# sandialabs/calibr8

Hardware: AMD Instinct MI355X
Metric: element Jacobian assemblies/sec, 1M hex8 J2-plasticity fp64 (higher is better)
Workload: dtype f64

## Files before the change

### calibr8_amd/csrc/c8_assemble_node.hpp

```cpp
#pragma once

#include "c8_assemble_wave.hpp"

#ifdef C8_STAMPS
#define C8_NSTAMP(i) ex.stamp_node(ga.stamps, node, i)
#else
#define C8_NSTAMP(i)
#endif

namespace c8 {

template <class M, class = void> struct has_closed_form_rows : std::false_type {};
template <class M> struct has_closed_form_rows<M, std::enable_if_t<M::HAS_CLOSED_FORM_ROWS>> : std::true_type {};

template <class E, class ModelD, int MAXDEG, bool MANY> struct NodeShared {
  static constexpr int NR = ModelD::NROW;
  static constexpr int LDR = NR + 4;
  static_assert(LDR % 2 == 0 && (E::NP0 * LDR * 8) % 256 == 128, "record stride: 16-byte aligned, element groups 32 banks apart");
  static constexpr int NREC = 8 * E::NP0 * LDR, NACC = MAXDEG * 16;
  alignas(16) double buf[MANY ? NREC + NACC : (NREC > NACC ? NREC : NACC)];
  alignas(16) double nodal[8][E::NN][4];
  double nshape[8];
  double el[8][2];
  double bsum[4];
  C8_HD double* rec(int s, int pt) { return buf + (s * E::NP0 + pt) * LDR; }
  C8_HD double* img() { return buf + (MANY ? NREC : 0); }
  C8_HD static int img01(int deg) { return 9 * deg; }
  C8_HD static int img10(int deg) { return 12 * deg; }
  C8_HD static int img11(int deg) { return 15 * deg; }
};

C8_HD double const* at_byte(double const* p, int off) { return reinterpret_cast<double const*>(reinterpret_cast<char const*>(p) + off); }

constexpr int NODE_NXI = 7;
template <int MAXDEG> struct NodeLane {
  static constexpr int N00 = (9 * MAXDEG + 63) / 64, N01 = (3 * MAXDEG + 63) / 64;
  double J[16];
  double a00[N00], a01[N01], a10[N01], a11;
  double bold;
  double rs;
  double G[9], xo[NODE_NXI], w, h;
  int e, a, pos;
  bool valid;
};

template <class EX, class = void> struct has_xor8 : std::false_type {};
template <class EX> struct has_xor8<EX, std::void_t<typename EX::has_xor8>> : std::true_type {};
template <class EX, class = void> struct has_lane_marker : std::false_type {};
template <class EX> struct has_lane_marker<EX, std::void_t<decltype(std::declval<EX&>().cur)>> : std::true_type {};
template <int C, class EX, class F> C8_HD double lane_xor8(EX& ex, int lane, F get) {
  static_assert(C >= 0 && C < 8, "partner inside the group of eight lanes");
  if constexpr (C == 0) return get(lane);
  else if constexpr (has_xor8<EX>::value) return ex.template xor8<C>(lane, get);
  else if constexpr (has_lane_marker<EX>::value) {
    int const saved = ex.cur;
    ex.cur = lane ^ C;
    double const v = get(lane ^ C);
    ex.cur = saved;
    return v;
  } else return get(lane ^ C);
}

C8_HD constexpr int hex_code(int n) { return n ^ ((n >> 1) & 1); }
template <class E> C8_HD void hex_pattern(int j, double* v) {
  double c[3], w;
  E::point(0, 7, c, w);
  double const a = 1. + ((j & 1) ? c[0] : -c[0]), b = 1. + ((j & 2) ? c[1] : -c[1]), d = 1. + ((j & 4) ? c[2] : -c[2]);
  v[0] = 0.125 * a * b * d;
  v[1] = 0.125 * b * d;
  v[2] = 0.125 * a * d;
  v[3] = 0.125 * a * b;
}

template <class E> struct HexShape {
  double c[3];
  C8_HD static HexShape of_point(int pt) {
    double w;
    HexShape h;
    E::point(0, pt, h.c, w);
    return h;
  }
  C8_HD double at_node(int n) const {
    double const sx = ((n ^ (n >> 1)) & 1) ? 1. : -1., sy = ((n >> 1) & 1) ? 1. : -1., sz = ((n >> 2) & 1) ? 1. : -1.;
    return 0.125 * (1. + sx * c[0]) * (1. + sy * c[1]) * (1. + sz * c[2]);
  }
};

template <class E, template <class> class ModelT, int MAXDEG, bool MANY, bool ADJ = false, class EX>
C8_HD void node_rows_closed(EX& ex, NodeShared<E, ModelT<Dual>, MAXDEG, MANY>& sh, MeshTables const& mt, ModelSettings const& ms,
                            FieldArgs const& fa, GatherArgs const& ga, int node, AdjointArgs const& aa = AdjointArgs{}) {
  using Model = ModelT<Dual>;
  using SH = NodeShared<E, Model, MAXDEG, MANY>;
  using NL_ = NodeLane<MAXDEG>;
  constexpr int NL = Model::NLOC, NR = SH::NR;
  static_assert(NL <= NODE_NXI, "NodeLane::xo holds a point's local state");
  static_assert(E::NN == 8 && E::NP0 == 8 && E::SAME_POINTS, "row-per-node kernel: hex8-like element");
  static_assert(!Mechanics::USES_U && !Model::FINITE_DEF, "row-per-node kernel: small-strain weak form without u terms");
  C8_NSTAMP(6);
  int const nptr = ga.nodeptr[node], deg = ga.nodeptr[node + 1] - nptr;
  int const e0 = ga.nodeelem_ptr[node], e1 = ga.nodeelem_ptr[node + 1];
  size_t const np = (size_t)nptr;
  int const n3 = 3 * deg;
  if (e0 == e1) return;
  C8_NSTAMP(0);
  auto zero_acc = [&](int lane) {
    C8_UNROLL
    for (int it = 0; it < (SH::NACC + 63) / 64; ++it) {
      int const q = lane + 64 * it;
      if (q < 16 * deg) sh.img()[q] = 0.;
    }
    if (lane < 4) sh.bsum[lane] = 0.;
  };
  if (!ADJ || MANY) {
    ex.each([&](int lane) {
      if (!ADJ && lane < 8) {
        double v[4];
        hex_pattern<E>(lane, v);
        sh.nshape[lane] = v[0];
      }
      if (MANY) zero_acc(lane);
    });
    ex.sync();
  }
  for (int c0 = e0; c0 < e1; c0 += 8) {
    int const ne = (e1 - c0 < 8) ? e1 - c0 : 8;
    ex.each([&](int lane) {
      auto& r = ex.lane(lane);
      int const s = lane >> 3, m = lane & 7, mp = hex_code(m);
      r.valid = s < ne;
      r.rs = 0.;
      if (!r.valid) return;
      int const packed = ga.nodeelem[c0 + s];
      int const e = packed >> 3, a = packed & 7;
      r.e = e;
      r.a = a;
      int const nd = mt.conn[(size_t)e * E::NN + m];
      r.pos = ga.pos[((size_t)e * E::NN + m) * E::NN + a];
      {
        double const* const t = mt.shape + (size_t)e * SHAPE_STRIDE;
        C8_UNROLL
        for (int c = 0; c < 9; ++c) r.G[c] = t[SHAPE_JINV + 8 * c + mp];
        if constexpr (!ADJ) {
          size_t const q0 = ((size_t)e * E::NP0 + mp) * NL;
          C8_UNROLL
          for (int j = 0; j < NL; ++j) r.xo[j] = fa.xi_prev[q0 + j];
        }
        r.w = t[SHAPE_WDV + mp];
        r.h = t[SHAPE_H];
      }
      double* const nv = sh.nodal[s][m];
      nv[0] = fa.u[(size_t)nd * 3 + 0]; nv[1] = fa.u[(size_t)nd * 3 + 1]; nv[2] = fa.u[(size_t)nd * 3 + 2];
      nv[3] = fa.p[nd];
    });
    ex.sync();
    ex.each([&](int lane_) {
      auto& r = ex.lane(lane_);
      int lane = lane_;
      C8_PIN(lane);
      int const s = lane >> 3, pt = hex_code(lane & 7);
      if (!r.valid) return;
      int const e = r.e, a = r.a;
      size_t const q0 = ((size_t)e * E::NP0 + pt) * NL;
      double G[9], xi_old[NL];
      C8_UNROLL
      for (int c = 0; c < 9; ++c) G[c] = r.G[c];
      if constexpr (!ADJ) {
        C8_UNROLL
        for (int j = 0; j < NL; ++j) xi_old[j] = r.xo[j];
      }
      double fh4[4] = {0., 0., 0., 0.}, gx[NL];
      C8_UNROLL
      for (int j = 0; j < NL; ++j) gx[j] = 0.;
      if constexpr (ADJ) {
        double const* const fh = aa.f + ((size_t)e * E::NP0 + pt) * E::NDOF;
        fh4[0] = fh[3 * a + 0]; fh4[1] = fh[3 * a + 1]; fh4[2] = fh[3 * a + 2]; fh4[3] = fh[3 * E::NN + a];
        C8_UNROLL
        for (int j = 0; j < NL; ++j) gx[j] = aa.g[((size_t)e * E::NP0 + pt) * NL + j];
      }
      double q[WQ];
      C8_UNROLL
      for (int c = 0; c < WQ; ++c) q[c] = 0.;
      double g[3];
      {
        double R[12], pN = 0.;
        C8_UNROLL
        for (int c = 0; c < 12; ++c) R[c] = 0.;
        int const mo = hex_code(pt ^ 7) * 32;
        C8_UNROLL
        for (int i = 0; i < E::NN; ++i) {
          double v[4];
          hex_pattern<E>(i, v);
          double const t0 = (i & 1) ? v[1] : -v[1], t1 = (i & 2) ? v[2] : -v[2], t2 = (i & 4) ? v[3] : -v[3];
          double const* const nv = at_byte(sh.nodal[s][0], mo ^ (hex_code(i) * 32));
          double const u0 = nv[0], u1 = nv[1], u2 = nv[2], pm = nv[3];
          R[0] += u0 * t0; R[1] += u0 * t1; R[2] += u0 * t2;
          R[3] += u1 * t0; R[4] += u1 * t1; R[5] += u1 * t2;
          R[6] += u2 * t0; R[7] += u2 * t1; R[8] += u2 * t2;
          pN += pm * v[0];
          R[9] += pm * t0; R[10] += pm * t1; R[11] += pm * t2;
        }
        double const s0 = (pt & 1) ? 1. : -1., s1 = (pt & 2) ? 1. : -1., s2 = (pt & 4) ? 1. : -1.;
        C8_UNROLL
        for (int f = 0; f < 4; ++f) {
          double const r0 = s0 * R[3 * f], r1 = s1 * R[3 * f + 1], r2 = s2 * R[3 * f + 2];
          C8_UNROLL
          for (int d = 0; d < 3; ++d) q[(f < 3 ? 3 * f : 10) + d] = r0 * G[d] + r1 * G[3 + d] + r2 * G[6 + d];
        }
        q[9] = pN;
        double xa[3], wa, da[3];
        E::point(0, pt, xa, wa);
        E::dNdxi(a, xa, da);
        C8_UNROLL
        for (int d = 0; d < 3; ++d) g[d] = da[0] * G[d] + da[1] * G[3 + d] + da[2] * G[6 + d];
      }
      C8_NSTAMP(7);
      if constexpr (ADJ) {
        C8_UNROLL
        for (int j = 0; j < NL; ++j) xi_old[j] = fa.xi_prev[q0 + j];
      }
      int const es = mt.elem_set ? mt.elem_set[e] : 0;
      C8_UNROLL
      for (int c = 0; c < 9; ++c) r.G[c] = ((pt >> (c / 3)) & 1) ? G[c] : -G[c];
      typename Model::ClosedForm cf;
      Model::closed_form(mt.params + (size_t)es * Model::NPARAMS, q, xi_old, ms.abs_tol, r.h, ms.stab_mult, cf, true);
      if (!ADJ && a == 0) {
        C8_UNROLL
        for (int j = 0; j < NL; ++j) fa.xi[q0 + j] = cf.xi[j];
      }
      C8_NSTAMP(8);
      double const w = r.w;
      double Na;
      if constexpr (ADJ) Na = HexShape<E>::of_point(pt).at_node(a);
      else Na = sh.nshape[hex_code(a) ^ pt ^ 7];
      double* const rc = sh.rec(s, pt);
      double el[2];
      Model::template closed_form_row<ADJ>(cf.t, w, g, Na, rc, el);
      if (pt == 0) { sh.el[s][0] = el[0]; sh.el[s][1] = el[1]; }
      if constexpr (!ADJ) {
        C8_UNROLL
        for (int i = 0; i < 3; ++i) rc[NR + i] = w * (cf.F[3 * i] * g[0] + cf.F[3 * i + 1] * g[1] + cf.F[3 * i + 2] * g[2]);
        rc[NR + 3] = w * (cf.F[9] * Na + cf.F[10] * g[0] + cf.F[11] * g[1] + cf.F[12] * g[2]);
      } else {
        double Re[6];
        double dq[10];
        C8_UNROLL
        for (int k = 0; k < 10; ++k) dq[k] = 0.;
        if (aa.qoi.c_load != 0.) {
          double dxi[NL];
          Model::closed_form_load_term(mt.params + (size_t)es * Model::NPARAMS, aa.qoi.c_load * w, aa.qoi.comp,
                                       aa.qoi.S + ((size_t)e * E::NP0 + pt) * 3, dxi, dq);
          C8_UNROLL
          for (int j = 0; j < NL; ++j) gx[j] -= dxi[j];
        }
        Model::closed_form_adjoint(mt.params + (size_t)es * Model::NPARAMS, cf.t, gx, Re);
        double const dJ = aa.qoi.c_avg * w / aa.qoi.ndims * Na;
        rc[NR + 0] = (Re[0] - dq[0]) * g[0] + (Re[1] - dq[1]) * g[1] + (Re[2] - dq[2]) * g[2] - dJ + fh4[0];
        rc[NR + 1] = (Re[1] - dq[3]) * g[0] + (Re[3] - dq[4]) * g[1] + (Re[4] - dq[5]) * g[2] - dJ + fh4[1];
        rc[NR + 2] = (Re[2] - dq[6]) * g[0] + (Re[4] - dq[7]) * g[1] + (Re[5] - dq[8]) * g[2] - dJ + fh4[2];
        rc[NR + 3] = -dq[9] * Na + fh4[3];
      }
    });
    ex.sync();
    C8_NSTAMP(1);
    ex.each([&](int lane_) {
      auto& r = ex.lane(lane_);
      int lane = lane_;
      C8_PIN(lane);
      C8_UNROLL
      for (int j = 0; j < 16; ++j) r.J[j] = 0.;
      if (!r.valid) return;
      int const s = lane >> 3, m = lane & 7;
      double const el[2] = {sh.el[s][0], sh.el[s][1]};
      auto step = [&](auto cc) {
        constexpr int c = decltype(cc)::value, hc = hex_code(c);
        double v[4];
        hex_pattern<E>(hc ^ 7, v);
        double const k0 = (hc & 1) ? -v[1] : v[1], k1 = (hc & 2) ? -v[2] : v[2], k2 = (hc & 4) ? -v[3] : v[3];
        double h[3];
        C8_UNROLL
        for (int d = 0; d < 3; ++d)
          h[d] = lane_xor8<c>(ex, lane, [&](int l) -> double {
            double const* const Gs = ex.lane(l).G;
            return k0 * Gs[d] + k1 * Gs[3 + d] + k2 * Gs[6 + d];
          });
        Model::closed_form_block(sh.rec(s, hex_code(m) ^ hc), el, h, v[0], r.J);
        C8_UNROLL
        for (int j = 0; j < 16; ++j) C8_PIN(r.J[j]);
        C8_SCHED_FENCE();
      };
      step(std::integral_constant<int, 0>{}); step(std::integral_constant<int, 1>{});
      step(std::integral_constant<int, 2>{}); step(std::integral_constant<int, 3>{});
      step(std::integral_constant<int, 4>{}); step(std::integral_constant<int, 5>{});
      step(std::integral_constant<int, 6>{}); step(std::integral_constant<int, 7>{});
      if (m < 4) {
        double v = 0.;
        C8_UNROLL
        for (int pt = 0; pt < E::NP0; ++pt) v += sh.rec(s, pt)[NR + m];
        r.rs = v;
      }
    });
    C8_NSTAMP(2);
    if (c0 == e0) {
      ex.each([&](int lane_) {
        auto& r = ex.lane(lane_);
        int lane = lane_;
        C8_PIN(lane);
        C8_UNROLL
        for (int it = 0; it < NL_::N00; ++it) {
          int const j = lane + 64 * it;
          r.a00[it] = 0.;
          if (!ga.assign && j < 9 * deg) r.a00[it] = ga.A[0][0][np * 9 + j];
        }
        C8_UNROLL
        for (int it = 0; it < NL_::N01; ++it) {
          int const j = lane + 64 * it;
          r.a01[it] = r.a10[it] = 0.;
          if (!ga.assign && j < n3) { r.a01[it] = ga.A[0][1][np * 3 + j]; r.a10[it] = ga.A[1][0][np * 3 + j]; }
        }
        r.a11 = 0.;
        if (!ga.assign && lane < deg) r.a11 = ga.A[1][1][np + lane];
        r.bold = 0.;
        if (!ga.assign && lane < 4) r.bold = lane < 3 ? ga.b[0][(size_t)node * 3 + lane] : ga.b[1][node];
      });
    }
    if (!MANY) {
      ex.sync();
      ex.each([&](int lane) { zero_acc(lane); });
    }
    ex.sync();
    C8_NSTAMP(3);
    auto add_block = [&](int lane) {
      auto& r = ex.lane(lane);
      double* const c00 = sh.img() + 3 * r.pos;
      double* const c01 = sh.img() + SH::img01(deg) + r.pos;
      double* const c10 = sh.img() + SH::img10(deg) + 3 * r.pos;
      double* const c11 = sh.img() + SH::img11(deg) + r.pos;
      C8_UNROLL
      for (int j = 0; j < 16; ++j) {
        int const i = j >> 2, col = j & 3;
        ex.lds_add(i < 3 ? (col < 3 ? c00 + i * n3 + col : c01 + i * deg) : (col < 3 ? c10 + col : c11), r.J[j]);
      }
      if ((lane & 7) < 4) ex.lds_add(&sh.bsum[lane & 7], r.rs);
    };
#ifndef C8_TUNE_NODE_C_BY_ELEMENT
    ex.each([&](int lane) {
      if ((lane >> 3) >= ne) return;
      add_block(lane);
    });
#else
    for (int s2 = 0; s2 < ne; ++s2) {
      ex.each([&](int lane) {
        if ((lane >> 3) != s2) return;
        add_block(lane);
      });
    }
#endif
    ex.sync();
    C8_NSTAMP(4);
    if (!MANY) break;
  }
  ex.each([&](int lane_) {
    auto& r = ex.lane(lane_);
    int lane = lane_;
    C8_PIN(lane);
    C8_UNROLL
    for (int it = 0; it < NL_::N00; ++it) C8_PIN(r.a00[it]);
    C8_UNROLL
    for (int it = 0; it < NL_::N01; ++it) { C8_PIN(r.a01[it]); C8_PIN(r.a10[it]); }
    C8_PIN(r.a11);
    C8_PIN(r.bold);
    double const* const i00 = sh.img(), * const i01 = i00 + SH::img01(deg), * const i10 = i00 + SH::img10(deg), * const i11 = i00 + SH::img11(deg);
    C8_UNROLL
    for (int it = 0; it < NL_::N00; ++it) {
      int const j = lane + 64 * it;
      if (j < 9 * deg) ga.A[0][0][np * 9 + j] = r.a00[it] + i00[j];
    }
    C8_UNROLL
    for (int it = 0; it < NL_::N01; ++it) {
      int const j = lane + 64 * it;
      if (j < n3) {
        ga.A[0][1][np * 3 + j] = r.a01[it] + i01[j];
        ga.A[1][0][np * 3 + j] = r.a10[it] + i10[j];
      }
    }
    if (lane < deg) ga.A[1][1][np + lane] = r.a11 + i11[lane];
    if (lane < 3) ga.b[0][(size_t)node * 3 + lane] = r.bold + sh.bsum[lane];
    if (lane == 3) ga.b[1][node] = r.bold + sh.bsum[3];
  });
  ex.sync();
  C8_NSTAMP(5);
}

template <class E, template <class> class ModelT>
C8_HD void node_rows_update_g(MeshTables const& mt, AdjointArgs const& aa, size_t qp) {
  using Model = ModelT<Dual>;
  int const e = (int)(qp / E::NP0), pt = (int)(qp % E::NP0);
  int const es = mt.elem_set ? mt.elem_set[e] : 0;
  double const w = mt.shape[(size_t)e * SHAPE_STRIDE + SHAPE_WDV + pt];
  double dxi[Model::NLOC], dq[10];
  Model::closed_form_load_term(mt.params + (size_t)es * Model::NPARAMS, aa.qoi.c_load * w, aa.qoi.comp, aa.qoi.S + qp * 3, dxi, dq);
  C8_UNROLL
  for (int j = 0; j < Model::NLOC; ++j) aa.g[qp * Model::NLOC + j] -= dxi[j];
}

}
```

### calibr8_amd/csrc/c8_models.hpp

```cpp
#pragma once

#include "c8_math.hpp"

namespace c8 {

enum { C8_ELASTIC_PATH = 0, C8_PLASTIC_PATH = 1 };


C8_HD void set_val(double& x, double v) { x = v; }
C8_HD void set_val(Dual& x, double v) { x.v = v; }

template <class T> struct PointState {
  T u[3];
  T p;
  T grad_p[3];
  Tens3<T> grad_u;
  Tens3<T> grad_u_prev;
};

template <class T> C8_HD T compute_mu(T const& E, T const& nu) { return E / (2. * (1. + nu)); }
template <class T> C8_HD T compute_kappa(T const& E, T const& nu) { return E / (3. * (1. - 2. * nu)); }

template <class T> C8_HD Tens3<T> small_strain(Tens3<T> const& g) {
  Tens3<T> const gt = transpose(g);
// ... 89 lines not shown
  static constexpr int WAVE_BLOCKS_PER_CU = 2, WAVE_BLOCKS_PER_CU_ADJ = 2;
  static constexpr int WAVE_BLOCKS_PER_CU_K4 = 3;
  static constexpr bool GJ_XLANE_JAC = false, GJ_XLANE_K4 = true;
  static constexpr bool GJ_XLANE_NEWTON = true;
  static constexpr bool NEWTON_MATRIX_IN_LDS = false;
  using Trial = NoTrial;
  C8_HD Trial trial(PointState<T> const&) const { return {}; }
  C8_HD int evaluate(PointState<T> const& g, double abs_tol, Trial const&) { return evaluate(g, abs_tol); }
  T params[NPARAMS];
  T xi[NLOC], xi_prev[NLOC], R[NLOC];
  C8_HD static void init_variables(double* xi0) { C8_UNROLL for (int k = 0; k < NLOC; ++k) xi0[k] = 0.; }
  C8_HD void initial_guess(PointState<T> const&) {
    C8_UNROLL
    for (int k = 0; k < NLOC; ++k) set_val(xi[k], val(xi_prev[k]));
  }
  C8_HD Tens3<T> dev_cauchy(PointState<T> const& g) const {
    T const mu = compute_mu(params[0], params[1]);
    Tens3<T> const eps = small_strain(g.grad_u);
    Tens3<T> const pstrain = sym_dim<DIM>(xi);
    Tens3<T> const dev_eps = (DIM == 3) ? dev(eps) : minus_s_eye<DIM>(eps, trace(eps) * (1. / 3.));
    return scale(2. * mu, dev_eps - pstrain);
  }
  C8_HD Tens3<T> cauchy(PointState<T> const& g) const {
    return minus_s_eye<DIM>(dev_cauchy(g), g.p);
  }
  C8_HD T hydro_cauchy(PointState<T> const& g) const {
    T const E = params[0], nu = params[1];
    T const kappa = compute_kappa(E, nu);
    return kappa * trace(small_strain(g.grad_u)) - params[4] * params[5] * E / (1. - 2. * nu);
  }
  C8_HD T pressure_scale_factor() const { return compute_kappa(params[0], params[1]); }
  C8_HD int evaluate(PointState<T> const& g, double abs_tol, bool force_path = false, int path_in = 0) {
    double const sqrt_23 = 0.81649658092772603273;
    double const sqrt_32 = 1.22474487139158904910;
    T const mu = compute_mu(params[0], params[1]);
    T const K = params[2], Y = params[3];
    T const alpha = xi[NSYM], alpha_old = xi_prev[NSYM];
    Tens3<T> const s = dev_cauchy(g);
    T const s_mag = norm(s);
    T const sigma_yield = Y + K * alpha;
    T const f = (s_mag - sqrt_23 * sigma_yield) / val(mu);
    int path;
    if (!force_path) path = (val(f) > abs_tol || fabs(val(f)) < abs_tol) ? C8_PLASTIC_PATH : C8_ELASTIC_PATH;
    else path = path_in;
    if (path == C8_PLASTIC_PATH) {
      T const dgam = sqrt_32 * (alpha - alpha_old);
      T const c = dgam / s_mag;
      Tens3<T> const Rp = sym_dim<DIM>(xi) - sym_dim<DIM>(xi_prev) - scale(c, s);
      pack_sym_dim<DIM>(Rp, R);
      R[NSYM] = f;
    } else {
      C8_UNROLL
      for (int k = 0; k < NLOC; ++k) R[k] = xi[k] - xi_prev[k];
    }
    return path;
  }
  static constexpr bool HAS_CLOSED_FORM = (DIM == 3);
  struct ClosedForm {
    static constexpr int NT = 14;
    double xi[NLOC];
    double F[13];
    double t[NT];
  };
  C8_HD static void closed_form(double const* prm, double const* q, double const* xi_old, double abs_tol, double h,
                                double stab_mult, ClosedForm& cf, bool pressure_mass) {
    double const sqrt_23 = 0.81649658092772603273;
    double const E = prm[0], nu = prm[1], K = prm[2], Y = prm[3];
    double const mu = E * c8_rcp(2. * (1. + nu)), kappa = E * c8_rcp(3. * (1. - 2. * nu));
    double const inv_mu = c8_rcp(mu);
    double eps[9];
    C8_UNROLL
    for (int i = 0; i < 3; ++i)
      C8_UNROLL
      for (int j = 0; j < 3; ++j) eps[3 * i + j] = 0.5 * (q[3 * i + j] + q[3 * j + i]);
    double const tr = eps[0] + eps[4] + eps[8];
    double const th = tr * (1. / 3.);
    double const pold[9] = {xi_old[0], xi_old[1], xi_old[2], xi_old[1], xi_old[3], xi_old[4], xi_old[2], xi_old[4], xi_old[5]};
    double st[9], ss = 0.;
    C8_UNROLL
    for (int k = 0; k < 9; ++k) {
      double const dev = eps[k] - ((k == 0 || k == 4 || k == 8) ? th : 0.);
      st[k] = (2. * mu) * (dev - pold[k]);
      ss += st[k] * st[k];
    }
    double const smag = sqrt(ss);
    double const alpha_old = xi_old[NSYM];
    double const excess = smag - sqrt_23 * (Y + K * alpha_old);
    double const f0 = excess * inv_mu;
    bool const plastic = f0 > abs_tol || fabs(f0) < abs_tol;
    double theta = 1.;
    double* n = cf.t + 5;
    cf.t[1] = 0.;
    C8_UNROLL
    for (int k = 0; k < NLOC; ++k) cf.xi[k] = xi_old[k];
    C8_UNROLL
    for (int k = 0; k < 9; ++k) n[k] = 0.;
    cf.t[2] = 0.;
    if (plastic) {
      double const inv_H = c8_rcp(2. * mu + (2. / 3.) * K);
      double const dgam = fabs(f0) < abs_tol ? 0. : excess * inv_H;
      double const inv = c8_rcp(smag);
      C8_UNROLL
      for (int k = 0; k < 9; ++k) n[k] = st[k] * inv;
      cf.t[2] = (n[0] + n[4] + n[8]) * (1. / 3.);
      theta = 1. - (2. * mu) * dgam * inv;
      cf.t[1] = (2. * mu) * (1. - (2. * mu) * inv_H - theta);
      cf.xi[0] = xi_old[0] + dgam * n[0]; cf.xi[1] = xi_old[1] + dgam * n[1]; cf.xi[2] = xi_old[2] + dgam * n[2];
      cf.xi[3] = xi_old[3] + dgam * n[4]; cf.xi[4] = xi_old[4] + dgam * n[5]; cf.xi[5] = xi_old[5] + dgam * n[8];
      cf.xi[NSYM] = alpha_old + sqrt_23 * dgam;
    }
    cf.t[0] = (2. * mu) * theta;
    double const inv_kappa = c8_rcp(kappa);
    double const tau = (stab_mult * 0.5 * h * h) * inv_mu;
    cf.t[3] = pressure_mass ? inv_kappa : 0.;
    cf.t[4] = tau;
    double const p = q[9];
    C8_UNROLL
    for (int k = 0; k < 9; ++k) cf.F[k] = theta * st[k] - ((k == 0 || k == 4 || k == 8) ? p : 0.);
    double const hydro = kappa * tr - prm[4] * prm[5] * E * c8_rcp(1. - 2. * nu);
    cf.F[9] = pressure_mass ? -(hydro * inv_kappa) + -(p * inv_kappa) : -(hydro * inv_kappa);
    cf.F[10] = -(tau * q[10]); cf.F[11] = -(tau * q[11]); cf.F[12] = -(tau * q[12]);
  }
  C8_HD static void closed_form_flux_column(double const* t, double const* ek, double isp, double const* g, double N, double* db) {
    double const a = t[0], b = t[1], trn3 = t[2], inv_kappa = t[3], tau = t[4];
    double const* n = t + 5;
    double const gk = ek[0] * g[0] + ek[1] * g[1] + ek[2] * g[2];
    double ng[3];
    C8_UNROLL
    for (int i = 0; i < 3; ++i) ng[i] = n[3 * i] * g[0] + n[3 * i + 1] * g[1] + n[3 * i + 2] * g[2];
    double const nkg = ek[0] * ng[0] + ek[1] * ng[1] + ek[2] * ng[2];
    double const bnk = b * (nkg - trn3 * gk);
    double const Np = isp * N;
    double const diag = a * gk * (1. / 3.) + Np;
    double const ha = 0.5 * a;
    double hg[3], hek[3];
    C8_UNROLL
    for (int i = 0; i < 3; ++i) { hg[i] = ha * g[i]; hek[i] = ek[i]; }
    C8_UNROLL
    for (int i = 0; i < 3; ++i)
      C8_UNROLL
      for (int j = 0; j < 3; ++j) {
        double const v = hek[i] * hg[j] + hg[i] * hek[j] + n[3 * i + j] * bnk;
        db[3 * i + j] = (i == j) ? v - diag : v;
      }
    db[9] = -gk - Np * inv_kappa;
    double const tp = isp * tau;
    db[10] = -(tp * g[0]); db[11] = -(tp * g[1]); db[12] = -(tp * g[2]);
  }
  static constexpr bool HAS_CLOSED_FORM_ROWS = HAS_CLOSED_FORM;
  static constexpr int NROW = 14;
  template <bool TR = false>
  C8_HD static void closed_form_row(double const* t, double w, double const* g, double Na, double* r, double* el) {
    double const a = t[0], b = t[1], trn3 = t[2];
    double const* n = t + 5;
    r[0] = w * g[0]; r[1] = w * g[1]; r[2] = w * g[2];
    double const wb = w * b;
    double const ta = TR ? trn3 : 0., tb = TR ? 0. : trn3;
    C8_UNROLL
    for (int i = 0; i < 3; ++i) r[3 + i] = wb * (n[3 * i] * g[0] + n[3 * i + 1] * g[1] + n[3 * i + 2] * g[2] - ta * g[i]);
    r[6] = 0.5 * a;
    r[7] = w * Na;
    r[8] = n[0] - tb; r[9] = n[1]; r[10] = n[2]; r[11] = n[4] - tb; r[12] = n[5]; r[13] = n[8] - tb;
    el[0] = t[4];
    el[1] = t[3];
  }
  C8_HD static void closed_form_load_term(double const* prm, double wc, int c, double const* S, double* dJ_dxi, double* dJ_dq) {
    double const mu2 = prm[0] * c8_rcp(1. + prm[1]);
    double const Sc = c == 0 ? S[0] : (c == 1 ? S[1] : S[2]);
    double const k = wc * mu2;
    dJ_dxi[0] = -k * (c == 0 ? S[0] : 0.);
    dJ_dxi[1] = -k * (c == 0 ? S[1] : (c == 1 ? S[0] : 0.));
    dJ_dxi[2] = -k * (c == 0 ? S[2] : (c == 2 ? S[0] : 0.));
    dJ_dxi[3] = -k * (c == 1 ? S[1] : 0.);
    dJ_dxi[4] = -k * (c == 1 ? S[2] : (c == 2 ? S[1] : 0.));
    dJ_dxi[5] = -k * (c == 2 ? S[2] : 0.);
    dJ_dxi[NSYM] = 0.;
    C8_UNROLL
    for (int a = 0; a < 3; ++a)
      C8_UNROLL
      for (int l = 0; l < 3; ++l)
        dJ_dq[3 * a + l] = k * (0.5 * ((c == a ? S[l] : 0.) + (c == l ? S[a] : 0.)) - (a == l ? Sc * (1. / 3.) : 0.));
    dJ_dq[9] = -wc * Sc;
  }
  C8_HD static void closed_form_adjoint(double const* prm, double const* t, double const* gxi, double* Re) {
    double const sqrt_23 = 0.81649658092772603273;
    double const mu = prm[0] * c8_rcp(2. * (1. + prm[1]));
    double const i2mu = c8_rcp(2. * mu);
    double const a = t[0], b = t[1], trn3 = t[2];
    double const* n = t + 5;
    double const omt = 1. - a * i2mu;
    double const tmH = omt - b * i2mu;
    double const G[6] = {gxi[0], 0.5 * gxi[1], 0.5 * gxi[2], gxi[3], 0.5 * gxi[4], gxi[5]};
    double const Gn = G[0] * n[0] + G[3] * n[4] + G[5] * n[8] + 2. * (G[1] * n[1] + G[2] * n[2] + G[4] * n[5]);
    double const ca = -(b * i2mu) * Gn + gxi[NSYM] * sqrt_23 * tmH;
    double const trG3 = (G[0] + G[3] + G[5]) * (1. / 3.);
    Re[0] = ca * (n[0] - trn3) + omt * (G[0] - trG3);
    Re[1] = ca * n[1] + omt * G[1];
    Re[2] = ca * n[2] + omt * G[2];
    Re[3] = ca * (n[4] - trn3) + omt * (G[3] - trG3);
    Re[4] = ca * n[5] + omt * G[4];
    Re[5] = ca * (n[8] - trn3) + omt * (G[5] - trG3);
  }
  C8_HD static void closed_form_local_adjoint(double const* prm, double const* t, double wdv, double const* ZG, double const* g_in,
                                              double* phi, double* g_out) {
    static_assert(DIM == 3, "3-D form");
    double const sqrt_32 = 1.22474487139158904910, sqrt_6 = 2.44948974278317809820, sqrt_23 = 0.81649658092772603273;
    double const mu = prm[0] * c8_rcp(2. * (1. + prm[1]));
    double const c = 2. * mu * wdv;
    double const* nn = t + 5;
    double const n[6] = {nn[0], nn[1], nn[2], nn[4], nn[5], nn[8]};
    double v[NLOC];
    v[0] = g_in[0] + c * ZG[0];
    v[1] = g_in[1] + c * (ZG[1] + ZG[3]);
    v[2] = g_in[2] + c * (ZG[2] + ZG[6]);
    v[3] = g_in[3] + c * ZG[4];
    v[4] = g_in[4] + c * (ZG[5] + ZG[7]);
    v[5] = g_in[5] + c * ZG[8];
    v[NSYM] = g_in[NSYM];
    bool plastic = false;
    C8_UNROLL
    for (int k = 0; k < 9; ++k) plastic = plastic || (nn[k] != 0.);
    if (!plastic) {
      C8_UNROLL
      for (int k = 0; k < NLOC; ++k) { phi[k] = v[k]; g_out[k] = v[k]; }
      return;
    }
    double const theta = t[0] * c8_rcp(2. * mu);
    double const beta = (1. - theta) * c8_rcp(theta);
    double const kap = sqrt_23 * prm[2] * c8_rcp(mu);
    double nv = 0.;
    C8_UNROLL
    for (int k = 0; k < 6; ++k) nv += n[k] * v[k];
    double const pa = -(v[NSYM] + sqrt_32 * nv) * c8_rcp(sqrt_6 + kap);
    double const a = nv + 2. * pa;
    double const f = beta * a + 2. * pa;
    double const ib = c8_rcp(1. + beta);
    C8_UNROLL
    for (int k = 0; k < 6; ++k) {
      double const wk = (k == 1 || k == 2 || k == 4) ? 2. : 1.;
      phi[k] = (v[k] + wk * n[k] * f) * ib;
      g_out[k] = phi[k];
    }
    phi[NSYM] = pa;
    g_out[NSYM] = -sqrt_32 * a;
  }
  C8_HD static double closed_form_param_gradient(double const* prm, double const* q, double const* xi, double abs_tol, double h,
                                                 double stab_mult, double wdv, double const* ZG, double const* phi, int mine,
                                                 double wload, int comp, double const* S) {
    static_assert(DIM == 3, "3-D form");
    double const sqrt_23 = 0.81649658092772603273;
    double const E = prm[0], nu = prm[1], K = prm[2], Y = prm[3], cte = prm[4], dT = prm[5];
    double const mu = E * c8_rcp(2. * (1. + nu)), kappa = E * c8_rcp(3. * (1. - 2. * nu));
    double const dmu = mine == 0 ? mu * c8_rcp(E) : (mine == 1 ? -mu * c8_rcp(1. + nu) : 0.);
    double const dkap = mine == 0 ? kappa * c8_rcp(E) : (mine == 1 ? 2. * kappa * c8_rcp(1. - 2. * nu) : 0.);
    double const dK = mine == 2 ? 1. : 0., dY = mine == 3 ? 1. : 0., dcte = mine == 4 ? 1. : 0., ddT = mine == 5 ? 1. : 0.;
    double eps[9];
    C8_UNROLL
    for (int i = 0; i < 3; ++i)
      C8_UNROLL
      for (int j = 0; j < 3; ++j) eps[3 * i + j] = 0.5 * (q[3 * i + j] + q[3 * j + i]);
    double const th = (eps[0] + eps[4] + eps[8]) * (1. / 3.);
    double const ep[9] = {xi[0], xi[1], xi[2], xi[1], xi[3], xi[4], xi[2], xi[4], xi[5]};
    double D[9], dd = 0.;
    C8_UNROLL
    for (int k = 0; k < 9; ++k) {
      D[k] = eps[k] - ((k == 0 || k == 4 || k == 8) ? th : 0.) - ep[k];
      dd += D[k] * D[k];
    }
    double const smag = 2. * mu * sqrt(dd);
    double const alpha = xi[NSYM];
    double const f = (smag - sqrt_23 * (Y + K * alpha)) * c8_rcp(mu);
    bool const plastic = f > abs_tol || fabs(f) < abs_tol;
    double s = 0.;
    if (plastic) s = phi[NSYM] * (dmu * smag * c8_rcp(mu) - sqrt_23 * (dY + dK * alpha)) * c8_rcp(mu);
    double DZ = 0.;
    C8_UNROLL
    for (int k = 0; k < 9; ++k) DZ += D[k] * ZG[k];
    double const th3 = E * c8_rcp((1. - 2. * nu) * kappa);
    double const dVp = dkap * q[9] * c8_rcp(kappa * kappa) + (dcte * dT + ddT * cte) * th3;
    double const tau = (stab_mult * 0.5 * h * h) * c8_rcp(mu);
    double const dGp = dmu * tau * c8_rcp(mu);
    s += wdv * (2. * dmu * DZ + dVp * ZG[9] + dGp * (q[10] * ZG[10] + q[11] * ZG[11] + q[12] * ZG[12]));
    if (wload != 0.) s += 2. * dmu * wload * (D[3 * comp] * S[0] + D[3 * comp + 1] * S[1] + D[3 * comp + 2] * S[2]);
    return s;
  }
  C8_HD static void closed_form_block(double const* r, double const* el, double const* h, double Nm, double* J) {
    double const gh = r[0] * h[0] + r[1] * h[1] + r[2] * h[2];
    double const nh[3] = {r[8] * h[0] + r[9] * h[1] + r[10] * h[2], r[9] * h[0] + r[11] * h[1] + r[12] * h[2],
                          r[10] * h[0] + r[12] * h[1] + r[13] * h[2]};
    double const p1[3] = {r[6] * r[0], r[6] * r[1], r[6] * r[2]};
    double const m3 = r[6] * (-2. / 3.);
    double const p2[3] = {m3 * h[0], m3 * h[1], m3 * h[2]};
    C8_UNROLL
    for (int i = 0; i < 3; ++i)
      C8_UNROLL
      for (int k = 0; k < 3; ++k) J[4 * i + k] = fma(r[3 + i], nh[k], fma(r[i], p2[k], fma(p1[k], h[i], J[4 * i + k])));
    double const d = r[6] * gh;
    J[0] += d; J[5] += d; J[10] += d;
    C8_UNROLL
    for (int i = 0; i < 3; ++i) J[4 * i + 3] = fma(-r[i], Nm, J[4 * i + 3]);
    C8_UNROLL
    for (int k = 0; k < 3; ++k) J[12 + k] = fma(-r[7], h[k], J[12 + k]);
    J[15] = fma(-el[0], gh, fma(-(r[7] * el[1]), Nm, J[15]));
  }
};
template <class T> struct SmallJ2 : SmallJ2Dim<T, 3> {};
template <class T> struct SmallJ2Plane : SmallJ2Dim<T, 2> {};

template <class T> struct SmallHillPlaneStrain {
  static constexpr int NLOC = 4, NPARAMS = 9;
  static constexpr bool FINITE_DEF = false, HAS_LOCAL = true;
  static constexpr int WAVE_BLOCKS_PER_CU = 2, WAVE_BLOCKS_PER_CU_ADJ = 2;
  static constexpr int WAVE_BLOCKS_PER_CU_K4 = 2;
  static constexpr bool GJ_XLANE_JAC = false, GJ_XLANE_K4 = false;
  static constexpr bool NEWTON_MATRIX_IN_LDS = false;
  using Trial = NoTrial;
  C8_HD Trial trial(PointState<T> const&) const { return {}; }
  C8_HD int evaluate(PointState<T> const& g, double abs_tol, Trial const&) { return evaluate(g, abs_tol); }
  T params[NPARAMS];
  T xi[NLOC], xi_prev[NLOC], R[NLOC];
  C8_HD static void init_variables(double* xi0) { C8_UNROLL for (int k = 0; k < NLOC; ++k) xi0[k] = 0.; }
  C8_HD void initial_guess(PointState<T> const&) {
    C8_UNROLL
    for (int k = 0; k < NLOC; ++k) set_val(xi[k], val(xi_prev[k]));
  }
  C8_HD Tens3<T> dev_cauchy(PointState<T> const& g) const {
    T const mu = compute_mu(params[0], params[1]);
    Tens3<T> const eps = small_strain(g.grad_u);
    return scale(2. * mu, minus_s_eye<2>(eps, trace(eps) * (1. / 3.)) - sym_dim<2>(xi));
  }
  C8_HD Tens3<T> cauchy(PointState<T> const& g) const { return minus_s_eye<2>(dev_cauchy(g), g.p); }
  C8_HD T hydro_cauchy(PointState<T> const& g) const {
    return compute_kappa(params[0], params[1]) * trace(small_strain(g.grad_u));
  }
  C8_HD T pressure_scale_factor() const { return compute_kappa(params[0], params[1]); }
  C8_HD int evaluate(PointState<T> const& g, double abs_tol, bool force_path = false, int path_in = 0) {
    T const mu = compute_mu(params[0], params[1]);
    T const Y = params[2], S = params[3], D = params[4];
    auto inv2 = [](T const& r) { return 1. / (r * r); };
    T const i00 = inv2(params[5]), i11 = inv2(params[6]), i22 = inv2(params[7]);
    T const F = 0.5 * (i11 + i22 - i00), G = 0.5 * (i22 + i00 - i11), H = 0.5 * (i00 + i11 - i22);
    T const N = 1.5 * inv2(params[8]);
    T const alpha = xi[3], alpha_old = xi_prev[3];
    Tens3<T> const ps = sym_dim<2>(xi);
    Tens3<T> const s = dev_cauchy(g);
    T const s_zz = (2. * mu) * (-(trace(small_strain(g.grad_u)) * (1. / 3.)) + trace(ps));
    T const d12 = s.yy - s_zz, d20 = s_zz - s.xx, d01 = s.xx - s.yy;
    T const hill = c8_sqrt(F * d12 * d12 + G * d20 * d20 + H * d01 * d01 + 2. * (N * s.xy * s.xy));
    T const sigma_yield = Y + S * (1. - c8_exp(-(D * alpha)));
    T const f = (hill - sigma_yield) / val(mu);
    int path;
    if (!force_path) path = (val(f) > abs_tol || fabs(val(f)) < abs_tol) ? C8_PLASTIC_PATH : C8_ELASTIC_PATH;
    else path = path_in;
    if (path == C8_PLASTIC_PATH) {
      Tens3<T> n = scale(0., ps);
      n.xx = ((G + H) * s.xx - H * s.yy - G * s_zz) / hill;
      n.yy = ((F + H) * s.yy - H * s.xx - F * s_zz) / hill;
      n.xy = n.yx = N * s.xy / hill;
      T const dgam = alpha - alpha_old;
      pack_sym_dim<2>(ps - sym_dim<2>(xi_prev) - scale(dgam, n), R);
      R[3] = f;
    } else {
      C8_UNROLL
      for (int k = 0; k < NLOC; ++k) R[k] = xi[k] - xi_prev[k];
    }
    return path;
  }
};

template <class T> struct HyperJ2PlaneStrain {
  static constexpr int NLOC = 5, NPARAMS = 6;
  static constexpr bool FINITE_DEF = true, HAS_LOCAL = true;
  static constexpr int WAVE_BLOCKS_PER_CU = 2, WAVE_BLOCKS_PER_CU_ADJ = 2;
  static constexpr int WAVE_BLOCKS_PER_CU_K4 = 2;
  static constexpr bool GJ_XLANE_JAC = false, GJ_XLANE_K4 = false;
  static constexpr bool NEWTON_MATRIX_IN_LDS = false;
  T params[NPARAMS];
  T xi[NLOC], xi_prev[NLOC], R[NLOC];
  C8_HD static void init_variables(double* xi0) {
    C8_UNROLL
    for (int k = 0; k < NLOC; ++k) xi0[k] = 0.;
    xi0[3] = 1.;
  }
  struct Trial { T zeta_trial[3], Ie_trial; };
  C8_HD Trial trial(PointState<T> const& g) const {
    Tens3<T> const I = eye3<T>();
    Tens3<T> const rF = matmul(g.grad_u + I, inverse(g.grad_u_prev + I));
    T const det_rF_13 = c8_cbrt(det(rF));
    Tens3<T> const rF_bar = scale(1. / det_rF_13, rF);
    Tens3<T> inner = sym_dim<2>(xi_prev);
    inner.xx = inner.xx + xi_prev[3];
    inner.yy = inner.yy + xi_prev[3];
    Tens3<T> const be2 = matmul(matmul(rF_bar, inner), transpose(rF_bar));
    T const zeta_zz = -(xi_prev[0] + xi_prev[2]);
    T const be_zz = (zeta_zz + xi_prev[3]) / (det_rF_13 * det_rF_13);
    Trial t;
    t.Ie_trial = (be2.xx + be2.yy + be_zz) / 3.;
    t.zeta_trial[0] = be2.xx - t.Ie_trial;
    t.zeta_trial[1] = be2.xy;
    t.zeta_trial[2] = be2.yy - t.Ie_trial;
    return t;
  }
  C8_HD void initial_guess(PointState<T> const& g) {
    Trial const t = trial(g);
    C8_UNROLL
    for (int k = 0; k < 3; ++k) set_val(xi[k], val(t.zeta_trial[k]));
    set_val(xi[3], val(t.Ie_trial));
    set_val(xi[4], val(xi_prev[4]));
  }
  C8_HD Tens3<T> dev_cauchy(PointState<T> const& g) const {
    T const mu = compute_mu(params[0], params[1]);
    T const J = det(g.grad_u + eye3<T>());
    return scale(mu / J, sym_dim<2>(xi));
  }
  C8_HD Tens3<T> cauchy(PointState<T> const& g) const { return minus_s_eye<2>(dev_cauchy(g), g.p); }
  C8_HD T hydro_cauchy(PointState<T> const& g) const {
    T const kappa = compute_kappa(params[0], params[1]);
    T const J = det(g.grad_u + eye3<T>());
    return (kappa * 0.5) * (J - 1. / J);
  }
  C8_HD T pressure_scale_factor() const { return compute_kappa(params[0], params[1]); }
  C8_HD int evaluate(PointState<T> const& g, double abs_tol, bool force_path = false, int path_in = 0) {
    return evaluate(g, abs_tol, trial(g), force_path, path_in);
  }
  C8_HD int evaluate(PointState<T> const& g, double abs_tol, Trial const& tr, bool force_path = false, int path_in = 0) {
    double const sqrt_23 = 0.81649658092772603273;
    double const sqrt_32 = 1.22474487139158904910;
    T const mu = compute_mu(params[0], params[1]);
    T const K = params[2], Y = params[3], Y_inf = params[4], delta = params[5];
    T const Ie = xi[3], alpha = xi[4], alpha_old = xi_prev[4];
    Tens3<T> const zeta = sym_dim<2>(xi);
    T const zeta_zz = -(xi[0] + xi[2]);
    Tens3<T> s3 = scale(mu, zeta);
    s3.zz = mu * zeta_zz;
    T const s_mag = norm(s3);
    T const sigma_yield = Y + K * alpha + (Y_inf - Y) * (1. - c8_exp(-(delta * alpha)));
    T const f = (s_mag - sqrt_23 * sigma_yield) / val(mu);
    int path;
    if (!force_path) path = (val(f) > abs_tol || fabs(val(f)) < abs_tol) ? C8_PLASTIC_PATH : C8_ELASTIC_PATH;
    else path = path_in;
    Tens3<T> Rz = zeta - sym_dim<2>(tr.zeta_trial);
    if (path == C8_PLASTIC_PATH) {
      T const dgam = sqrt_32 * (alpha - alpha_old);
      T const c = (2. * dgam) * Ie * mu / s_mag;
      Rz = Rz + scale(c, zeta);
      Tens3<T> be = zeta;
      be.xx = be.xx + Ie; be.yy = be.yy + Ie; be.zz = zeta_zz + Ie;
      R[3] = det(be) - 1.;
      R[4] = f;
    } else {
      R[3] = Ie - tr.Ie_trial;
      R[4] = alpha - alpha_old;
    }
    pack_sym_dim<2>(Rz, R);
    return path;
  }
};

template <class T> struct SmallHill {
  static constexpr bool PIN_PHASES_K1 = false, PIN_PHASES_K3 = true;
  static constexpr int NLOC = 7, NPARAMS = 11;
  static constexpr bool FINITE_DEF = false, HAS_LOCAL = true;
  static constexpr int WAVE_BLOCKS_PER_CU = 2, WAVE_BLOCKS_PER_CU_ADJ = 2;
  static constexpr int WAVE_BLOCKS_PER_CU_K4 = 2;
  static constexpr bool GJ_XLANE_JAC = false, GJ_XLANE_K4 = true;
  static constexpr bool NEWTON_MATRIX_IN_LDS = false;
  using Trial = NoTrial;
  C8_HD Trial trial(PointState<T> const&) const { return {}; }
  C8_HD int evaluate(PointState<T> const& g, double abs_tol, Trial const&) { return evaluate(g, abs_tol); }
  T params[NPARAMS];
  T xi[NLOC], xi_prev[NLOC], R[NLOC];
  C8_HD static void init_variables(double* xi0) { C8_UNROLL for (int k = 0; k < NLOC; ++k) xi0[k] = 0.; }
  C8_HD void initial_guess(PointState<T> const&) {
    C8_UNROLL
    for (int k = 0; k < NLOC; ++k) set_val(xi[k], val(xi_prev[k]));
  }
  C8_HD Tens3<T> dev_cauchy(PointState<T> const& g) const {
    T const mu = compute_mu(params[0], params[1]);
    Tens3<T> const eps = small_strain(g.grad_u);
    Tens3<T> const pstrain = sym6(xi);
    return scale(2. * mu, dev(eps) - pstrain);
  }
  C8_HD Tens3<T> cauchy(PointState<T> const& g) const {
    Tens3<T> s = dev_cauchy(g);
    s.xx = s.xx - g.p; s.yy = s.yy - g.p; s.zz = s.zz - g.p;
    return s;
  }
  C8_HD T hydro_cauchy(PointState<T> const& g) const {
    return compute_kappa(params[0], params[1]) * trace(small_strain(g.grad_u));
  }
  C8_HD T pressure_scale_factor() const { return compute_kappa(params[0], params[1]); }
  C8_HD int evaluate(PointState<T> const& g, double abs_tol, bool force_path = false, int path_in = 0) {
    T const mu = compute_mu(params[0], params[1]);
    T const Y = params[2], S = params[9], D = params[10];
    auto inv2 = [](T const& r) { return 1. / (r * r); };
    T const i00 = inv2(params[3]), i11 = inv2(params[4]), i22 = inv2(params[5]);
    T const F = 0.5 * (i11 + i22 - i00), G = 0.5 * (i22 + i00 - i11), H = 0.5 * (i00 + i11 - i22);
    T const L = 1.5 * inv2(params[8]), M = 1.5 * inv2(params[7]), N = 1.5 * inv2(params[6]);
    T const alpha = xi[6], alpha_old = xi_prev[6];
    Tens3<T> const s = dev_cauchy(g);
    T const d12 = s.yy - s.zz, d20 = s.zz - s.xx, d01 = s.xx - s.yy;
    T const hill = c8_sqrt(F * d12 * d12 + G * d20 * d20 + H * d01 * d01 +
                           2. * (L * s.yz * s.yz + M * s.xz * s.xz + N * s.xy * s.xy));
    T const sigma_yield = Y + S * (1. - c8_exp(-(D * alpha)));
    T const f = (hill - sigma_yield) / val(mu);
    int path;
    if (!force_path) path = (val(f) > abs_tol || fabs(val(f)) < abs_tol) ? C8_PLASTIC_PATH : C8_ELASTIC_PATH;
    else path = path_in;
    if (path == C8_PLASTIC_PATH) {
      Tens3<T> n;
      n.xx = ((G + H) * s.xx - H * s.yy - G * s.zz) / hill;
      n.yy = ((F + H) * s.yy - H * s.xx - F * s.zz) / hill;
      n.zz = ((G + F) * s.zz - G * s.xx - F * s.yy) / hill;
      n.xy = n.yx = N * s.xy / hill;
      n.xz = n.zx = M * s.xz / hill;
      n.yz = n.zy = L * s.yz / hill;
      T const dgam = alpha - alpha_old;
      Tens3<T> const ps = sym6(xi);
      Tens3<T> Rp = ps - sym6(xi_prev) - scale(dgam, n);
      Rp.zz = trace(ps);
      pack_sym6(Rp, R);
      R[6] = f;
    } else {
      C8_UNROLL
      for (int k = 0; k < NLOC; ++k) R[k] = xi[k] - xi_prev[k];
    }
    return path;
  }
};

template <class T> struct HypoHill {
  static constexpr bool PIN_PHASES_K1 = true, PIN_PHASES_K3 = true;
  static constexpr int NLOC = 7, NPARAMS = 11;
  static constexpr bool FINITE_DEF = true, HAS_LOCAL = true;
#ifndef C8_TUNE_HH_WAVES
#define C8_TUNE_HH_WAVES 2
#endif
  static constexpr int WAVE_BLOCKS_PER_CU = C8_TUNE_HH_WAVES, WAVE_BLOCKS_PER_CU_ADJ = 1;
  static constexpr int WAVE_BLOCKS_PER_CU_K4 = 1;
  static constexpr bool GJ_XLANE_JAC = false, GJ_XLANE_K4 = false;
#ifdef C8_TUNE_HH_NEWTON_LDS
  static constexpr bool NEWTON_MATRIX_IN_LDS = true;
#else
  static constexpr bool NEWTON_MATRIX_IN_LDS = false;
#endif
  T params[NPARAMS];
  T xi[NLOC], xi_prev[NLOC], R[NLOC];
  C8_HD static void init_variables(double* xi0) { C8_UNROLL for (int k = 0; k < NLOC; ++k) xi0[k] = 0.; }
  struct Trial { T d[6]; };
  C8_HD Trial trial(PointState<T> const& g) const {
    Tens3<T> const I = eye3<T>();
    Tens3<T> const F = g.grad_u + I;
    Tens3<T> const F_prev = g.grad_u_prev + I;
    Tens3<T> const Rot = polar_rotation(F);
    Tens3<T> const L = matmul(F - F_prev, inverse(F));
    Tens3<T> const D = scale(0.5, L + transpose(L));
    Trial t;
    pack_sym6(matmul(matmul(transpose(Rot), D), Rot), t.d);
    return t;
  }
  C8_HD void initial_guess(PointState<T> const& g) {
    double const E = val(params[0]), nu = val(params[1]);
    double const lambda = compute_lambda(E, nu), mu = compute_mu(E, nu);
    Trial const t = trial(g);
    double const ltr = lambda * (val(t.d[0]) + val(t.d[3]) + val(t.d[5]));
    C8_UNROLL
    for (int k = 0; k < 6; ++k) set_val(xi[k], val(xi_prev[k]) + 2. * mu * val(t.d[k]) + ((k == 0 || k == 3 || k == 5) ? ltr : 0.));
    set_val(xi[6], val(xi_prev[6]));
  }
  C8_HD Tens3<T> rotated_cauchy(PointState<T> const& g) const {
    Tens3<T> const Rot = polar_rotation(g.grad_u + eye3<T>());
    return matmul(matmul(Rot, sym6(xi)), transpose(Rot));
  }
  C8_HD Tens3<T> dev_cauchy(PointState<T> const& g) const { return dev(rotated_cauchy(g)); }
  C8_HD Tens3<T> cauchy(PointState<T> const& g) const {
    Tens3<T> s = dev_cauchy(g);
    s.xx = s.xx - g.p; s.yy = s.yy - g.p; s.zz = s.zz - g.p;
    return s;
  }
  C8_HD T hydro_cauchy(PointState<T> const& g) const { return trace(rotated_cauchy(g)) / 3.; }
  C8_HD void cauchy_and_hydro(PointState<T> const& g, Tens3<T>& sigma, T& sigma_h) const {
    Tens3<T> const RC = rotated_cauchy(g);
    sigma_h = trace(RC) / 3.;
    sigma = dev(RC);
    sigma.xx = sigma.xx - g.p; sigma.yy = sigma.yy - g.p; sigma.zz = sigma.zz - g.p;
  }
  C8_HD T pressure_scale_factor() const { return compute_kappa(params[0], params[1]); }
  C8_HD int evaluate(PointState<T> const& g, double abs_tol, bool force_path = false, int path_in = 0) {
    return evaluate(g, abs_tol, trial(g), force_path, path_in);
  }
  C8_HD int evaluate(PointState<T> const& g, double abs_tol, Trial const& tr, bool force_path = false, int path_in = 0) {
    T const lambda = compute_lambda(params[0], params[1]);
    T const mu = compute_mu(params[0], params[1]);
    T const Y = params[2], S = params[9], D = params[10];
    auto inv2 = [](T const& r) { return 1. / (r * r); };
    T const i00 = inv2(params[3]), i11 = inv2(params[4]), i22 = inv2(params[5]);
    T const F = 0.5 * (i11 + i22 - i00), G = 0.5 * (i22 + i00 - i11), H = 0.5 * (i00 + i11 - i22);
    T const L = 1.5 * inv2(params[8]), M = 1.5 * inv2(params[7]), N = 1.5 * inv2(params[6]);
    T const alpha = xi[6], alpha_old = xi_prev[6];
    Tens3<T> const TC = sym6(xi);
    T const d12 = TC.yy - TC.zz, d20 = TC.zz - TC.xx, d01 = TC.xx - TC.yy;
    T const hill = c8_sqrt(F * d12 * d12 + G * d20 * d20 + H * d01 * d01 +
                           2. * (L * TC.yz * TC.yz + M * TC.xz * TC.xz + N * TC.xy * TC.xy));
    T const sigma_yield = Y + S * (1. - c8_exp(-(D * alpha)));
    T const f = (hill - sigma_yield) / val(mu);
    Tens3<T> const d = sym6(tr.d);
// ... 976 lines not shown
```

Baseline: 303.1 million.

## Accumulate factored partial sums across corners, finish Jacobian block once

Result: faster. 320.9 million, median of 6 (+5.9%).

```diff
diff --git a/calibr8_amd/csrc/c8_assemble_node.hpp b/calibr8_amd/csrc/c8_assemble_node.hpp
--- a/calibr8_amd/csrc/c8_assemble_node.hpp
+++ b/calibr8_amd/csrc/c8_assemble_node.hpp
@@ -223,6 +223,8 @@
       for (int c = 0; c < 9; ++c) r.G[c] = ((pt >> (c / 3)) & 1) ? G[c] : -G[c];
       typename Model::ClosedForm cf;
       Model::closed_form(mt.params + (size_t)es * Model::NPARAMS, q, xi_old, ms.abs_tol, r.h, ms.stab_mult, cf, true);
+      double esc[2];
+      Model::closed_form_block_scalars(mt.params + (size_t)es * Model::NPARAMS, cf.t, esc);
       if (!ADJ && a == 0) {
         C8_UNROLL
         for (int j = 0; j < NL; ++j) fa.xi[q0 + j] = cf.xi[j];
@@ -235,7 +237,7 @@
       double* const rc = sh.rec(s, pt);
       double el[2];
       Model::template closed_form_row<ADJ>(cf.t, w, g, Na, rc, el);
-      if (pt == 0) { sh.el[s][0] = el[0]; sh.el[s][1] = el[1]; }
+      if (pt == 0) { sh.el[s][0] = esc[0]; sh.el[s][1] = esc[1]; }
       if constexpr (!ADJ) {
         C8_UNROLL
         for (int i = 0; i < 3; ++i) rc[NR + i] = w * (cf.F[3 * i] * g[0] + cf.F[3 * i + 1] * g[1] + cf.F[3 * i + 2] * g[2]);
@@ -266,11 +268,10 @@
       auto& r = ex.lane(lane_);
       int lane = lane_;
       C8_PIN(lane);
-      C8_UNROLL
-      for (int j = 0; j < 16; ++j) r.J[j] = 0.;
       if (!r.valid) return;
       int const s = lane >> 3, m = lane & 7;
-      double const el[2] = {sh.el[s][0], sh.el[s][1]};
+      double S[Model::NSUM];
+      double const rho = sh.el[s][0];
       auto step = [&](auto cc) {
         constexpr int c = decltype(cc)::value, hc = hex_code(c);
         double v[4];
@@ -283,15 +284,16 @@
             double const* const Gs = ex.lane(l).G;
             return k0 * Gs[d] + k1 * Gs[3 + d] + k2 * Gs[6 + d];
           });
-        Model::closed_form_block(sh.rec(s, hex_code(m) ^ hc), el, h, v[0], r.J);
-        C8_UNROLL
-        for (int j = 0; j < 16; ++j) C8_PIN(r.J[j]);
+        Model::template closed_form_block_sums<c == 0>(sh.rec(s, hex_code(m) ^ hc), rho, h, v[0], S);
+        C8_UNROLL
+        for (int j = 0; j < Model::NSUM; ++j) C8_PIN(S[j]);
         C8_SCHED_FENCE();
       };
       step(std::integral_constant<int, 0>{}); step(std::integral_constant<int, 1>{});
       step(std::integral_constant<int, 2>{}); step(std::integral_constant<int, 3>{});
       step(std::integral_constant<int, 4>{}); step(std::integral_constant<int, 5>{});
       step(std::integral_constant<int, 6>{}); step(std::integral_constant<int, 7>{});
+      Model::closed_form_block_finish(S, sh.el[s][1], r.J);
       if (m < 4) {
         double v = 0.;
         C8_UNROLL
diff --git a/calibr8_amd/csrc/c8_models.hpp b/calibr8_amd/csrc/c8_models.hpp
--- a/calibr8_amd/csrc/c8_models.hpp
+++ b/calibr8_amd/csrc/c8_models.hpp
@@ -415,6 +415,53 @@
     C8_UNROLL
     for (int k = 0; k < 3; ++k) J[12 + k] = fma(-r[7], h[k], J[12 + k]);
     J[15] = fma(-el[0], gh, fma(-(r[7] * el[1]), Nm, J[15]));
+  }
+  static constexpr int NSUM = 25;
+  C8_HD static void closed_form_block_scalars(double const* prm, double const* t, double* es) {
+    double const kappa = prm[0] * c8_rcp(3. * (1. - 2. * prm[1]));
+    es[0] = t[4] * kappa;
+    es[1] = t[3];
+  }
+  template <bool FIRST = false>
+  C8_HD static void closed_form_block_sums(double const* r, double rho, double const* h, double Nm, double* S) {
+    double const gh = r[0] * h[0] + r[1] * h[1] + r[2] * h[2];
+    double const nh[3] = {r[8] * h[0] + r[9] * h[1] + r[10] * h[2], r[9] * h[0] + r[11] * h[1] + r[12] * h[2],
+                          r[10] * h[0] + r[12] * h[1] + r[13] * h[2]};
+    double const p1[3] = {r[6] * r[0], r[6] * r[1], r[6] * r[2]};
+    if constexpr (FIRST) {
+      C8_UNROLL
+      for (int i = 0; i < 3; ++i)
+        C8_UNROLL
+        for (int k = 0; k < 3; ++k) { S[3 * i + k] = r[3 + i] * nh[k]; S[9 + 3 * k + i] = p1[k] * h[i]; }
+      C8_UNROLL
+      for (int i = 0; i < 3; ++i) { S[18 + i] = -r[i] * Nm; S[21 + i] = -r[7] * h[i]; }
+      S[24] = fma(rho, gh, r[7] * Nm);
+    } else {
+      C8_UNROLL
+      for (int i = 0; i < 3; ++i)
+        C8_UNROLL
+        for (int k = 0; k < 3; ++k) {
+          S[3 * i + k] = fma(r[3 + i], nh[k], S[3 * i + k]);
+          S[9 + 3 * k + i] = fma(p1[k], h[i], S[9 + 3 * k + i]);
+        }
+      C8_UNROLL
+      for (int i = 0; i < 3; ++i) { S[18 + i] = fma(-r[i], Nm, S[18 + i]); S[21 + i] = fma(-r[7], h[i], S[21 + i]); }
+      S[24] = fma(rho, gh, fma(r[7], Nm, S[24]));
+    }
+  }
+  C8_HD static void closed_form_block_finish(double const* S, double inv_kappa, double* J) {
+    double const* const X = S + 9;
+    double const tr = X[0] + X[4] + X[8];
+    C8_UNROLL
+    for (int i = 0; i < 3; ++i)
+      C8_UNROLL
+      for (int k = 0; k < 3; ++k) {
+        double const v = S[3 * i + k] + fma(-2. / 3., X[3 * i + k], X[3 * k + i]);
+        J[4 * i + k] = (i == k) ? v + tr : v;
+      }
+    C8_UNROLL
+    for (int i = 0; i < 3; ++i) { J[4 * i + 3] = S[18 + i]; J[12 + i] = S[21 + i]; }
+    J[15] = -(S[24] * inv_kappa);
   }
 };
 template <class T> struct SmallJ2 : SmallJ2Dim<T, 3> {};
```
